# CVMI-Lab/HybridNeuralRendering

Measured on AMD Instinct MI355X. Metric: rays/sec (fwd render) scene0241_01 at 1/2/4/8 GPU; PSNR delta vs ref, higher is better.
Workload: dtype f32

## Files before the change

### hybridneuralrendering_amd/csrc/hnr_h2.h

```cpp
#pragma once
#include <type_traits>

#include "hnr_common.h"

namespace hnr {

typedef float f32x16 __attribute__((ext_vector_type(16)));
typedef _Float16 f16x8 __attribute__((ext_vector_type(8)));
typedef unsigned int u32x4 __attribute__((ext_vector_type(4)));

constexpr int CH_ACT_EXP = 15;
constexpr int CH_W_EXP = 14;

__device__ __forceinline__ void split2h(float x0, float x1, unsigned &ph, unsigned &pm)
{
    float r0, r1;
    asm("v_cvt_pk_f16_f32 %0, %1, %2" : "=v"(ph) : "v"(x0), "v"(x1));
    asm("v_fma_mix_f32 %0, -%1, 1.0, %2 op_sel_hi:[1,0,0]" : "=v"(r0) : "v"(ph), "v"(x0));
    asm("v_fma_mix_f32 %0, -%1, 1.0, %2 op_sel:[1,0,0] op_sel_hi:[1,0,0]" : "=v"(r1) : "v"(ph), "v"(x1));
    asm("v_cvt_pk_f16_f32 %0, %1, %2" : "=v"(pm) : "v"(r0), "v"(r1));
}

__device__ __forceinline__ float pow2f(int e) { return __uint_as_float((unsigned)(127 + e) << 23); }

// ... 38 lines not shown
        for (int s = 0; s < PD && s < S; ++s) load_w(s, s);
    }
    __builtin_amdgcn_sched_barrier(0);
    mid();
    __builtin_amdgcn_sched_barrier(0);
    load_b(0, 0);
#pragma unroll
    for (int s = 0; s < S; ++s) {
        if (PACE == 0) {
            if (!PRELOAD_ALL && s + PD < S) load_w((s + PD) % (PD + 1), s + PD);
            if (s + 1 < S) load_b((s + 1) & 1, s + 1);
        }
        if (s == (PRELOAD_ALL || S <= PD ? 0 : S - 1 - PD)) { __builtin_amdgcn_sched_barrier(0); after(); __builtin_amdgcn_sched_barrier(0); }
        const int ws = PRELOAD_ALL ? s : s % (PD + 1), bs = s & 1;
#define CH_W(c, p) __builtin_bit_cast(f16x8, wf[ws][c][p])
#define CH_X(rt, p) __builtin_bit_cast(f16x8, bf[bs][rt][p])
        if (PACE > 0) {
            const bool has_b = s + 1 < S, has_w = !PRELOAD_ALL && s + PD < S;
#pragma unroll
            for (int m = 0; m < 3 * RT * CT; ++m) {
                const int term = m / (RT * CT), rt = (m % (RT * CT)) / CT, c = m % CT;
                const int wp = term == 0 ? 1 : 0, xp = term == 1 ? 1 : 0;
                acc[rt][c] = __builtin_amdgcn_mfma_f32_32x32x16_f16(CH_W(c, wp), CH_X(rt, xp), acc[rt][c], 0, 0, 0);
                bool load = false;
                if (has_b && m < 2 * RT) {
                    const int r2 = m >> 1, p2 = m & 1;
                    bf[(s + 1) & 1][r2][p2] = *reinterpret_cast<const u32x4 *>(bp + (s + 1) * SLOT + (r2 * 2 + p2) * 1024);
                    load = true;
                } else if (has_w && m >= 2 * RT && m < 2 * RT + 2 * CT) {
                    const int i2 = m - 2 * RT, c2 = i2 >> 1, p2 = i2 & 1;
                    wf[(s + PD) % (PD + 1)][c2][p2] = __builtin_bit_cast(u32x4, __builtin_amdgcn_raw_buffer_load_b128(wsrd, woff + (c2 * 2 + p2) * 1024, wbase + (WSAME ? 0 : s + PD) * WSTEP, 0));
                    load = true;
                }
                if (load) asm volatile("s_nop %0" :: "n"(PACE > 1 ? PACE - 2 : 0)); else asm volatile("s_nop %0" :: "n"(PACE > 0 ? PACE - 1 : 0));
                __builtin_amdgcn_sched_barrier(0);
            }
        } else {
#pragma unroll
        for (int rt = 0; rt < RT; ++rt)
#pragma unroll
            for (int c = 0; c < CT; ++c) acc[rt][c] = __builtin_amdgcn_mfma_f32_32x32x16_f16(CH_W(c, 1), CH_X(rt, 0), acc[rt][c], 0, 0, 0);
#pragma unroll
        for (int rt = 0; rt < RT; ++rt)
#pragma unroll
            for (int c = 0; c < CT; ++c) acc[rt][c] = __builtin_amdgcn_mfma_f32_32x32x16_f16(CH_W(c, 0), CH_X(rt, 1), acc[rt][c], 0, 0, 0);
#pragma unroll
// ... 21 lines not shown
```

### hybridneuralrendering_amd/csrc/mlp.hip

```cpp
#include <stdlib.h>

#include "hnr_h2.h"

namespace hnr {

constexpr int ML_PAD = 32;
constexpr int ML_SLOT = 8192 + ML_PAD;
constexpr int ML_WSTEP = 8192;
constexpr int ML_META_FLOATS = 4 * 128 + 4 + 4;
constexpr int ML_DESC = 4 * 128, ML_WMAX = 4 * 128 + 4;

struct MlpArgs {
    const float *A; int lda;
    const float *R; const int32_t *ridx; int ldr;
    const char *wimg;
    int wbase[4];
    int K0, N[4], act[4];
    float *C2; int ldc2;
    const float *loc_w; const int32_t *vs_item;
    const float *w2c, *Kmat, *campos, *campos_n;
    const float *fm; int H, W;
    const float *frame_w;
    const float *w_last, *b_last;
    const float *CF; int ldcf;
// ... 4 lines not shown
    float *C; int ldc;
    float *T0; int ldt0; float *T1; int ldt1;
    unsigned *tmax;
};

typedef float f32x4m __attribute__((ext_vector_type(4)));

#ifdef HNR_MLP_PROBE
__device__ long long g_mlp_probe[24];
#define MLP_STAMP(i_) do { const long long t_ = clock64(); tm_[i_] += t_ - tp_; tp_ = t_; if ((i_) == 0) ++ntile_; } while (0)
#else
#define MLP_STAMP(i_) do { } while (0)
#endif
constexpr int mlp3_wgs_per_cu(int S0, int RT, int MODE) { return MODE == 1 ? (RT >= 4 ? 2 : 4) : RT >= 4 ? 1 : (RT == 1 || S0 <= 6) ? 4 : 2; }

#ifdef HNR_MLP_FULL_BARRIER
#define MLP_LDS_BARRIER() __syncthreads()
#else
#define MLP_LDS_BARRIER() asm volatile("s_waitcnt lgkmcnt(0)\n\ts_barrier" ::: "memory")
#endif
#ifndef HNR_MLP_LPR16
#define HNR_MLP_LPR16 1
#endif
template <int S0, int S1, int S2, int S3, int MODE, int RT = 4>
__global__ __launch_bounds__(256, mlp3_wgs_per_cu(S0, RT, MODE)) void mlp3_kernel(MlpArgs a)
{
    static_assert(MODE != 1 || RT == 4 || RT == 2, "the merge stage is built on 128- or 64-row tiles (32 / 16 samples x 4 views)");
    constexpr int SLOT = RT * 2048 + ML_PAD, ROWS = 32 * RT;
    constexpr int SMAX3 = S0 > S1 ? (S0 > S2 ? S0 : S2) : (S1 > S2 ? S1 : S2), SMAX = SMAX3 > S3 ? SMAX3 : S3;
    extern __shared__ __attribute__((aligned(16))) char lds[];
    const int tid = threadIdx.x, lane = tid & 63, wave = tid >> 6, h = lane >> 5, j = lane & 31;
    long long M = a.M_cap;
    if (a.counts) { const long long c = (long long)a.counts[a.count_index] * a.count_mult; if (c < M) M = c; }
    long long n_unit = 1;
    if (a.seg_stride > 0) {
        n_unit = a.counts ? (long long)a.counts[a.count_index] : a.M_cap / (a.count_mult > 0 ? a.count_mult : 1);
        if (n_unit > a.seg_stride) n_unit = a.seg_stride;
        if (n_unit < 1) n_unit = 1;
        if (M > n_unit * a.count_mult) M = n_unit * a.count_mult;
    }
    auto phys = [&](long long m) -> long long {
        if (a.seg_stride <= 0) return m;
        int q = 0;
        for (int v = 1; v < a.count_mult && v < 8; ++v) q += (m >= (long long)v * n_unit) ? 1 : 0;
        return (long long)q * a.seg_stride + (m - (long long)q * n_unit);
    };
    const int n_tiles = (int)((M + ROWS - 1) / ROWS);
// ... 231 lines not shown
                }
            }
            __syncthreads();
        };
        auto store = [&](float *C, int ldc) {
#pragma unroll
            for (int rt = 0; rt < RTW; ++rt) {
                const long long row = row_base + 32 * (rt0 + rt) + j;
                if (row < M) {
                    float *o = C + (size_t)phys(row) * ldc + col0;
#pragma unroll
                    for (int q = 0; q < 4; ++q) {
                        const int c = col0 + 4 * q;
                        if (c + 4 <= ldc)
                            *reinterpret_cast<float4 *>(o + 4 * q) = make_float4(acc[rt][0][4 * q], acc[rt][0][4 * q + 1], acc[rt][0][4 * q + 2], acc[rt][0][4 * q + 3]);
                    }
                }
            }
        };
        const bool act0 = 32 * cw < a.N[0], act1 = 32 * cw < a.N[1], act2 = 32 * cw < a.N[2];
        float amax[RTW];
        zero_acc();
        if (act0) {
            h2_mfma_layer<RTW, 1, S0, 0, ML_WSTEP, SLOT>(wsrd, a.wbase[0], woff, lds_b, lane, acc, []() {}, [&]() { if (MODE == 1) { load_addend(0); load_addend(1); } });
            MLP_STAMP(3);
            if (a.R) activate(0, amax, std::true_type{}); else activate(0, amax, std::false_type{});
            MLP_STAMP(4);
            if (MODE == 0 && a.T0) {
                store(a.T0, a.ldt0);
#pragma unroll
                for (int rt = 0; rt < RTW; ++rt) tmax_run[0] = fmaxf(tmax_run[0], amax[rt]);
            }
        }
        publish(1, act0, amax);
        MLP_STAMP(5);
        zero_acc();
        if (act1) {
            h2_mfma_layer<RTW, 1, S1, 0, ML_WSTEP, SLOT>(wsrd, a.wbase[1], woff, lds_b, lane, acc, []() {});
            MLP_STAMP(6);
            activate(1, amax, std::false_type{});
            if (MODE == 0 && a.T1) {
                store(a.T1, a.ldt1);
#pragma unroll
                for (int rt = 0; rt < RTW; ++rt) tmax_run[1] = fmaxf(tmax_run[1], amax[rt]);
            }
        }
        publish(2, act1, amax);
        MLP_STAMP(7);
        float cfv[6] = {0.f, 0.f, 0.f, 0.f, 0.f, 0.f};
        float4 wl4[4];
        zero_acc();
        if (act2) {
            h2_mfma_layer<RTW, 1, S2, 0, ML_WSTEP, SLOT>(wsrd, a.wbase[2], woff, lds_b, lane, acc, []() {});
            MLP_STAMP(8);
            activate(2, amax, std::false_type{});
            MLP_STAMP(9);
            if (MODE != 1) store(a.C, a.ldc);
            if (MODE == 0 && a.tmax) {
#pragma unroll
                for (int rt = 0; rt < RTW; ++rt) tmax_run[2] = fmaxf(tmax_run[2], amax[rt]);
            }
            MLP_STAMP(10);
        }
        if (MODE == 1) {
#pragma unroll
            for (int it = 0; it < (8 * RT * 45 + 255) / 256; ++it) {
                const int idx = tid_t + 256 * it, ls = idx / 45, ch = idx - ls * 45;
                const long long sidx = row_base / 4 + ls;
                cfv[it] = (idx < 8 * RT * 45 && sidx * 4 < M) ? a.CF[(size_t)sidx * a.ldcf + ch] : 0.f;
            }
#pragma unroll
            for (int q4 = 0; q4 < 4; ++q4) wl4[q4] = *reinterpret_cast<const float4 *>(s_wl + col0 + 4 * q4);
        }
        if (MODE == 1) {
#pragma unroll
            for (int rt = 0; rt < RTW; ++rt) {
// ... 19 lines not shown
            MLP_LDS_BARRIER();
            MLP_STAMP(15);
            {
#pragma unroll
                for (int it = 0; it < (8 * RT * 45 + 255) / 256; ++it) {
                    const int idx = tid_t + 256 * it, ls = idx / 45, ch = idx - ls * 45;
                    const long long sidx = row_base / 4 + ls;
                    if (idx < 8 * RT * 45 && sidx * 4 < M) {
                        float fsum = 0.f, wsum = 0.f;
#pragma unroll
                        for (int v = 0; v < 4; ++v) { const float wv = s_w[4 * ls + v]; fsum += s_f[(4 * ls + v) * 48 + ch] * wv; wsum += wv; }
                        float *o = a.X7 + (size_t)sidx * a.ld7;
                        __builtin_nontemporal_store(cfv[it], o + ch);
                        __builtin_nontemporal_store(hnr_div(fsum, wsum + 1e-6f), o + 45 + ch);
                    }
                }
                MLP_STAMP(17);
            }
        }
        if (S3 > 0) {
            publish(3, act2, amax);
            zero_acc();
            if (32 * wave < a.N[3]) {
                h2_mfma_layer<RTW, 1, (S3 > 0 ? S3 : 1), 0, ML_WSTEP, SLOT>(wsrd, a.wbase[3], woff, lds_b, lane, acc, []() {});
                activate(3, amax, std::false_type{});
                store(a.C2, a.ldc2);
            }
        }
        MLP_STAMP(11);
        __syncthreads();
        MLP_STAMP(12);
    }
    if (MODE == 0 && a.tmax) {
        __syncthreads();
#pragma unroll
        for (int l = 0; l < 3; ++l) {
            float m = tmax_run[l];
            for (int o = 32; o > 0; o >>= 1) m = fmaxf(m, __shfl_xor(m, o));
            if (lane == 0) exch[4 * l + wave] = m;
        }
        __syncthreads();
        if (tid < 3) { const float m = fmaxf(fmaxf(exch[4 * tid], exch[4 * tid + 1]), fmaxf(exch[4 * tid + 2], exch[4 * tid + 3])); if (m > 0.f) atomicMax(a.tmax + tid, __float_as_uint(m)); }
    }
#ifdef HNR_MLP_PROBE
    if (blockIdx.x == 0 && threadIdx.x == 0) { for (int i = 0; i < 20; ++i) g_mlp_probe[i] = tm_[i]; g_mlp_probe[20] = ntile_; }
#endif
}

constexpr int MW_SLOT = 2048 + ML_PAD;
constexpr int MW_WAVE_LDS = 4 * MW_SLOT + 4 * 32 * 4 + 32 * 3 * 4;
constexpr int MW_WAVES = 12;
constexpr int MW_WBYTES = 11 * 4096;
constexpr int MW_SHARED = MW_WBYTES + 3 * 64 * 4 + 64 * 4 + 128 * 4;
constexpr int MW_LDS = MW_SHARED + MW_WAVES * MW_WAVE_LDS;
#define MW_WAVE_FENCE() asm volatile("s_waitcnt lgkmcnt(0)" ::: "memory")
template <int S>
__device__ __forceinline__ void mw_layer(const char *wp, const char *bp, f32x16 (&acc)[2])
{
    u32x4 wf[2][2][2], bf[2][2];
    auto ld = [&](int slot, int s) {
#pragma unroll
        for (int c = 0; c < 2; ++c)
#pragma unroll
            for (int q = 0; q < 2; ++q) wf[slot][c][q] = *reinterpret_cast<const u32x4 *>(wp + s * 4096 + (c * 2 + q) * 1024);
#pragma unroll
        for (int q = 0; q < 2; ++q) bf[slot][q] = *reinterpret_cast<const u32x4 *>(bp + s * MW_SLOT + q * 1024);
    };
    ld(0, 0);
#pragma unroll
    for (int s = 0; s < S; ++s) {
        if (s + 1 < S) ld((s + 1) & 1, s + 1);
        const int b = s & 1;
#define MW_W(c, q) __builtin_bit_cast(f16x8, wf[b][c][q])
#define MW_X(q) __builtin_bit_cast(f16x8, bf[b][q])
#pragma unroll
        for (int c = 0; c < 2; ++c) acc[c] = __builtin_amdgcn_mfma_f32_32x32x16_f16(MW_W(c, 1), MW_X(0), acc[c], 0, 0, 0);
#pragma unroll
        for (int c = 0; c < 2; ++c) acc[c] = __builtin_amdgcn_mfma_f32_32x32x16_f16(MW_W(c, 0), MW_X(1), acc[c], 0, 0, 0);
#pragma unroll
        for (int c = 0; c < 2; ++c) acc[c] = __builtin_amdgcn_mfma_f32_32x32x16_f16(MW_W(c, 0), MW_X(0), acc[c], 0, 0, 0);
#undef MW_W
#undef MW_X
    }
}

__global__ __launch_bounds__(64 * MW_WAVES, 1) void merge_wp_kernel(MlpArgs a)
{
    extern __shared__ __attribute__((aligned(16))) char lds[];
    const int tid = threadIdx.x, wave = __builtin_amdgcn_readfirstlane(tid >> 6);
    long long M = a.M_cap;
    if (a.counts) { const long long c = (long long)a.counts[a.count_index] * a.count_mult; if (c < M) M = c; }
    const long long n_samp = M / 4;
    const int n_tiles = (int)((n_samp + 7) / 8);
    const float *meta = reinterpret_cast<const float *>(a.wimg + (size_t)11 * ML_WSTEP);
    float *s_bias = reinterpret_cast<float *>(lds + MW_WBYTES);
    float *s_wl = s_bias + 3 * 64;
    float *s_cam = s_wl + 64;
    char *wl = lds + MW_SHARED + wave * MW_WAVE_LDS;
    int *s_pix = reinterpret_cast<int *>(wl + 4 * MW_SLOT);
    float *s_vm = reinterpret_cast<float *>(s_pix + 32), *s_w = s_vm + 32;
    unsigned *s_max = reinterpret_cast<unsigned *>(s_w + 32);
    float *s_dd = reinterpret_cast<float *>(s_max + 32);
    for (int i = tid; i < MW_WBYTES / 16; i += 64 * MW_WAVES) {
        const int s = i >> 8, cp = (i >> 6) & 3, ln = i & 63;
        *reinterpret_cast<u32x4 *>(lds + i * 16) = *reinterpret_cast<const u32x4 *>(a.wimg + (size_t)s * ML_WSTEP + cp * 1024 + ln * 16);
    }
    for (int i = tid; i < 3 * 64; i += 64 * MW_WAVES) s_bias[i] = meta[(i >> 6) * 128 + (i & 63)];
    for (int i = tid; i < 64; i += 64 * MW_WAVES) { s_wl[i] = a.w_last[i]; s_cam[i] = a.w2c[i]; }
    if (tid < 9) s_cam[64 + tid] = a.Kmat[tid];
    if (tid < 3) s_cam[76 + tid] = a.campos[tid];
    if (tid < 12) s_cam[80 + tid] = a.campos_n[tid];
    __syncthreads();
    const float dw0 = meta[ML_DESC + 0], dw1 = meta[ML_DESC + 1], dw2 = meta[ML_DESC + 2], b_last = a.b_last[0];
    const f32x2 slope2 = {a.slope, a.slope};
    for (int tile = blockIdx.x * MW_WAVES + wave; tile < n_tiles; tile += gridDim.x * MW_WAVES) {
        int lane = tid & 63;
        asm volatile("" : "+v"(lane));
        const int h = lane >> 5, j = lane & 31;
        const long long sbase = (long long)tile * 8;
        {
            const int ls = j >> 2, v = j & 3;
            long long sidx = sbase + ls;
// ... 67 lines not shown
            constexpr bool ADD = decltype(with_addend)::value;
            float m = 0.f;
            const f32x2 inv2 = {inv, inv};
#pragma unroll
            for (int c = 0; c < 2; ++c) {
#pragma unroll
                for (int q4 = 0; q4 < 4; ++q4) {
                    const float4 b = *reinterpret_cast<const float4 *>(s_bias + layer * 64 + 32 * c + 16 * h + 4 * q4);
#pragma unroll
                    for (int e = 0; e < 2; ++e) {
                        const int q = 2 * q4 + e;
                        f32x2 add = e ? f32x2{b.z, b.w} : f32x2{b.x, b.y};
                        if (ADD) { const float4 t4 = ad[c][q4]; add = add + (e ? f32x2{t4.z, t4.w} : f32x2{t4.x, t4.y}); }
                        f32x2 v = f32x2_fma(f32x2{acc[c][2 * q], acc[c][2 * q + 1]}, inv2, add);
                        const f32x2 sv = v * slope2;
                        v.x = fmaxf(v.x, sv.x); v.y = fmaxf(v.y, sv.y);
                        acc[c][2 * q] = v.x; acc[c][2 * q + 1] = v.y;
                        m = fmaxf(fmaxf(m, fabsf(v.x)), fabsf(v.y));
                    }
                }
            }
            return m;
        };
        auto publish = [&](float dw, float m) {
            m = fmaxf(m, __shfl_xor(m, 32));
            const int k = row_scale_exp(m);
            const float sc = pow2f(k);
            const f32x2 sc2 = {sc, sc};
            inv = __fmul_rn(pow2f(-k), dw);
            MW_WAVE_FENCE();
#pragma unroll
            for (int c = 0; c < 2; ++c) {
                unsigned ph[8], pm[8];
#pragma unroll
                for (int q = 0; q < 8; ++q) {
                    const f32x2 vs = f32x2{acc[c][2 * q], acc[c][2 * q + 1]} * sc2;
                    split2h(vs.x, vs.y, ph[q], pm[q]);
                }
                char *dst = wl + (2 * c + h) * MW_SLOT + j * 16;
                *reinterpret_cast<u32x4 *>(dst) = u32x4{ph[0], ph[1], ph[2], ph[3]};
                *reinterpret_cast<u32x4 *>(dst + 512) = u32x4{ph[4], ph[5], ph[6], ph[7]};
                *reinterpret_cast<u32x4 *>(dst + 1024) = u32x4{pm[0], pm[1], pm[2], pm[3]};
                *reinterpret_cast<u32x4 *>(dst + 1024 + 512) = u32x4{pm[4], pm[5], pm[6], pm[7]};
            }
            MW_WAVE_FENCE();
        };
        const char *wp = lds + lane * 16, *bp = wl + lane * 16;
        zero_acc();
        mw_layer<3>(wp, bp, acc);
        publish(dw1, activate(0, std::true_type{}));
        zero_acc();
        mw_layer<4>(wp + 3 * 4096, bp, acc);
        publish(dw2, activate(1, std::false_type{}));
        zero_acc();
        mw_layer<4>(wp + 7 * 4096, bp, acc);
        (void)activate(2, std::false_type{});
        {
            float d2[2];
#pragma unroll
            for (int c = 0; c < 2; ++c) {
                float d = 0.f;
#pragma unroll
                for (int q4 = 0; q4 < 4; ++q4) {
                    const float4 w4 = *reinterpret_cast<const float4 *>(s_wl + 32 * c + 16 * h + 4 * q4);
                    d = fmaf(acc[c][4 * q4], w4.x, d); d = fmaf(acc[c][4 * q4 + 1], w4.y, d);
                    d = fmaf(acc[c][4 * q4 + 2], w4.z, d); d = fmaf(acc[c][4 * q4 + 3], w4.w, d);
                }
                d2[c] = __fadd_rn(d, __shfl_xor(d, 32));
            }
            const float d = __fadd_rn(d2[0], d2[1]);
            float wv = hnr_div(1.f, 1.f + expf(-(d + b_last)));
            wv *= s_vm[j];
            if (a.frame_w) wv *= a.frame_w[j & 3];
            if (h == 0) s_w[j] = wv;
        }
        MW_WAVE_FENCE();
        float *s_x7 = reinterpret_cast<float *>(wl);
#pragma unroll
// ... 32 lines not shown
                __builtin_nontemporal_store(v, reinterpret_cast<f32x4m *>(a.X7 + (size_t)sidx * a.ld7 + 4 * c4));
            }
        }
        MW_WAVE_FENCE();
    }
}

struct MixArgs {
    const float *X7; int ld7;
    const char *wimg;
    const float *CF; int ldcf;
    const float *w_fin, *b_fin;
    const float *sigma; const int32_t *vs_item;
    const unsigned long long *counts; long long S_cap;
    float slope;
    float *Y; int ldy;
    float *decoded;
};
constexpr int MX_WAVES = 12;
constexpr int MX_WAVE_LDS = 3 * MW_SLOT + 32 * 4;
constexpr int MX_WBYTES = 12 * 4096;
constexpr int MX_SHARED = MX_WBYTES + 3 * 64 * 4 + 3 * 128 * 4;
constexpr int MX_LDS = MX_SHARED + MX_WAVES * MX_WAVE_LDS;
__global__ __launch_bounds__(64 * MX_WAVES, 1) void mixfinal_wp_kernel(MixArgs a)
{
    extern __shared__ __attribute__((aligned(16))) char lds[];
    const int tid = threadIdx.x, wave = __builtin_amdgcn_readfirstlane(tid >> 6);
    long long n_samp = a.S_cap;
    if (a.counts) { const long long c = (long long)a.counts[HNR_CNT_SAMPLES_VALID]; if (c < n_samp) n_samp = c; }
    const int n_tiles = (int)((n_samp + 31) / 32);
    const float *meta = reinterpret_cast<const float *>(a.wimg + (size_t)12 * ML_WSTEP);
    float *s_bias = reinterpret_cast<float *>(lds + MX_WBYTES);
    float *s_fin = s_bias + 3 * 64;
    char *wl = lds + MX_SHARED + wave * MX_WAVE_LDS;
    unsigned *s_max = reinterpret_cast<unsigned *>(wl + 3 * MW_SLOT);
    for (int i = tid; i < MX_WBYTES / 16; i += 64 * MX_WAVES) {
        const int s = i >> 8, cp = (i >> 6) & 3, ln = i & 63;
        *reinterpret_cast<u32x4 *>(lds + i * 16) = *reinterpret_cast<const u32x4 *>(a.wimg + (size_t)s * ML_WSTEP + cp * 1024 + ln * 16);
    }
    for (int i = tid; i < 3 * 64; i += 64 * MX_WAVES) s_bias[i] = meta[(i >> 6) * 128 + (i & 63)];
    for (int i = tid; i < 3 * 128; i += 64 * MX_WAVES) s_fin[i] = a.w_fin[i];
    __syncthreads();
    const float dw0 = meta[ML_DESC + 0], dw1 = meta[ML_DESC + 1], dw2 = meta[ML_DESC + 2];
    const float bfin[3] = {a.b_fin[0], a.b_fin[1], a.b_fin[2]};
    const f32x2 slope2 = {a.slope, a.slope};
    for (int tile = blockIdx.x * MX_WAVES + wave; tile < n_tiles; tile += gridDim.x * MX_WAVES) {
        int lane = tid & 63;
        asm volatile("" : "+v"(lane));
// ... 46 lines not shown
                for (int r = 0; r < 16; ++r) acc[c][r] = 0.f;
        };
        auto activate = [&](int layer, bool act) -> float {
            float m = 0.f;
            const f32x2 inv2 = {inv, inv};
#pragma unroll
            for (int c = 0; c < 2; ++c) {
#pragma unroll
                for (int q4 = 0; q4 < 4; ++q4) {
                    const float4 b = *reinterpret_cast<const float4 *>(s_bias + layer * 64 + 32 * c + 16 * h + 4 * q4);
#pragma unroll
                    for (int e = 0; e < 2; ++e) {
                        const int q = 2 * q4 + e;
                        const f32x2 add = e ? f32x2{b.z, b.w} : f32x2{b.x, b.y};
                        f32x2 v = f32x2_fma(f32x2{acc[c][2 * q], acc[c][2 * q + 1]}, inv2, add);
                        if (act) { const f32x2 sv = v * slope2; v.x = fmaxf(v.x, sv.x); v.y = fmaxf(v.y, sv.y); }
                        acc[c][2 * q] = v.x; acc[c][2 * q + 1] = v.y;
                        m = fmaxf(fmaxf(m, fabsf(v.x)), fabsf(v.y));
                    }
                }
            }
            return m;
        };
        auto publish = [&](float dw, float m) {
            m = fmaxf(m, __shfl_xor(m, 32));
            const int k = row_scale_exp(m);
            const float sc = pow2f(k);
            const f32x2 sc2 = {sc, sc};
            inv = __fmul_rn(pow2f(-k), dw);
            MW_WAVE_FENCE();
#pragma unroll
            for (int c = 0; c < 2; ++c) {
                unsigned ph[8], pm[8];
#pragma unroll
                for (int q = 0; q < 8; ++q) {
                    const f32x2 vs = f32x2{acc[c][2 * q], acc[c][2 * q + 1]} * sc2;
                    split2h(vs.x, vs.y, ph[q], pm[q]);
                }
                if (2 * c + h < 3) {
                    char *dst = wl + (2 * c + h) * MW_SLOT + j * 16;
                    *reinterpret_cast<u32x4 *>(dst) = u32x4{ph[0], ph[1], ph[2], ph[3]};
                    *reinterpret_cast<u32x4 *>(dst + 512) = u32x4{ph[4], ph[5], ph[6], ph[7]};
                    *reinterpret_cast<u32x4 *>(dst + 1024) = u32x4{pm[0], pm[1], pm[2], pm[3]};
                    *reinterpret_cast<u32x4 *>(dst + 1024 + 512) = u32x4{pm[4], pm[5], pm[6], pm[7]};
                }
            }
            MW_WAVE_FENCE();
        };
        const char *wp = lds + lane * 16, *bp = wl + lane * 16;
        long long srow = sbase + j;
        const bool ok = srow < n_samp;
        if (!ok) srow = n_samp - 1;
        zero_acc();
        mw_layer<3>(wp, bp, acc);
        MW_WAVE_FENCE();
        planes_half(1);
        MW_WAVE_FENCE();
        mw_layer<3>(wp + 3 * 4096, bp, acc);
        publish(dw1, activate(0, true));
        zero_acc();
        mw_layer<3>(wp + 6 * 4096, bp, acc);
        publish(dw2, activate(1, true));
        const float *cfrow = a.CF + (size_t)srow * a.ldcf;
        float4 cfa[2][4], cfb[8];
#pragma unroll
        for (int c = 0; c < 2; ++c)
#pragma unroll
            for (int q4 = 0; q4 < 4; ++q4) cfa[c][q4] = *reinterpret_cast<const float4 *>(cfrow + 32 * c + 16 * h + 4 * q4);
#pragma unroll
        for (int q4 = 0; q4 < 8; ++q4) cfb[q4] = *reinterpret_cast<const float4 *>(cfrow + 64 + 32 * h + 4 * q4);
        zero_acc();
        mw_layer<3>(wp + 9 * 4096, bp, acc);
        (void)activate(2, false);
        if (a.Y && ok) {
            float *o = a.Y + (size_t)srow * a.ldy;
#pragma unroll
            for (int c = 0; c < 2; ++c)
#pragma unroll
                for (int q4 = 0; q4 < 4; ++q4) {
                    const int col = 32 * c + 16 * h + 4 * q4;
                    if (col + 4 <= 48) *reinterpret_cast<float4 *>(o + col) = make_float4(acc[c][4 * q4], acc[c][4 * q4 + 1], acc[c][4 * q4 + 2], acc[c][4 * q4 + 3]);
                }
        }
        float x[2][16];
#pragma unroll
        for (int c = 0; c < 2; ++c)
#pragma unroll
            for (int r = 0; r < 16; ++r) {
                const float cfv = reinterpret_cast<const float *>(&cfa[c][0])[r];
                x[c][r] = (32 * c + 16 * h + r < 45) ? acc[c][r] + cfv : cfv;
            }
        float rj[3];
#pragma unroll
        for (int o = 0; o < 3; ++o) {
            const float *wf = s_fin + o * 128;
// ... 70 lines not shown
    for (int i = blockIdx.x * blockDim.x + threadIdx.x; i < total; i += gridDim.x * blockDim.x) {
        const int e = i & 7, ln = (i >> 3) & 63, ct = (i >> 9) & 3, s = i >> 11;
        const int ii = ln & 31, hh = ln >> 5;
        const int n = 32 * ct + 16 * ((ii >> 2) & 1) + (ii & 3) + 4 * (ii >> 3), k = 16 * s + 8 * hh + e;
        const float x = (n < a.N[l] && k < a.K[l]) ? __fmul_rn(a.W[l][(size_t)n * a.ldw[l] + k], scale) : 0.f;
        const _Float16 hv = (_Float16)x;
        const _Float16 mv = (_Float16)__fsub_rn(x, (float)hv);
        _Float16 *dst = reinterpret_cast<_Float16 *>(a.out + a.base[l] + (size_t)s * ML_WSTEP + (ct * 2) * 1024 + ln * 16) + e;
        dst[0] = hv;
        dst[512] = mv;
    }
    if (blockIdx.x == 0) {
        for (int i = threadIdx.x; i < 128; i += blockDim.x) meta[l * 128 + i] = (a.b[l] && i < a.N[l]) ? a.b[l][i] : 0.f;
        if (threadIdx.x == 0) meta[ML_DESC + l] = pow2f(-sw);
    }
}

}

using namespace hnr;

static int mlp_steps(int K) { return (K + 15) / 16; }

extern "C" int64_t hnr_mlp3_packed_bytes(int n_layers, const int *K)
{
    if (!K || (n_layers != 3 && n_layers != 4)) return -1;
    int64_t steps = 0;
    for (int l = 0; l < n_layers; ++l) { if (K[l] <= 0 || K[l] > 288) return -1; steps += mlp_steps(K[l]); }
    return steps * ML_WSTEP + ML_META_FLOATS * 4;
}

extern "C" int hnr_mlp3_pack(int n_layers, const float *const *d_W, const int *ldw, const int *N, const int *K, const float *const *d_bias, void *d_packed,
                             void *stream)
{
    if ((n_layers != 3 && n_layers != 4) || !d_W || !ldw || !N || !K || !d_bias || !d_packed || ((uintptr_t)d_packed & 15)) { set_error("hnr_mlp3_pack: NULL / unaligned pointer or n_layers not 3 / 4"); return HNR_ERR_BADARG; }
    MlpPackArgs a;
    int steps = 0;
    for (int l = 0; l < n_layers; ++l) {
        if (!d_W[l] || N[l] <= 0 || N[l] > 128 || K[l] <= 0 || K[l] > 288 || ldw[l] < K[l] || (l > 0 && K[l] != N[l == 3 ? 2 : l - 1])) {
            set_error("hnr_mlp3_pack: layer %d: N=%d (1..128) K=%d (1..288, = N of the layer it reads) ldw=%d", l, N[l], K[l], ldw[l]);
            return HNR_ERR_BADARG;
        }
        a.W[l] = d_W[l]; a.ldw[l] = ldw[l]; a.N[l] = N[l]; a.K[l] = K[l]; a.S[l] = mlp_steps(K[l]); a.b[l] = d_bias[l];
        a.base[l] = steps * ML_WSTEP;
        steps += a.S[l];
    }
// ... 63 lines not shown
    }
    if (M_cap == 0) return HNR_OK;
    if (!d_A || !d_packed || !d_C || ((uintptr_t)d_A & 15) || ((uintptr_t)d_C & 15) || ((uintptr_t)d_packed & 15) || ((uintptr_t)d_R & 7)) {
        set_error("hnr_mlp3_forward: NULL / unaligned pointer");
        return HNR_ERR_BADARG;
    }
    MlpArgs a;
    a.A = d_A; a.lda = lda; a.R = d_R; a.ridx = d_ridx; a.ldr = ldr; a.wimg = (const char *)d_packed;
    int steps = 0, S[4] = {0, 0, 0, 0};
    a.N[3] = 0; a.act[3] = 0; a.wbase[3] = 0;
    for (int l = 0; l < n_layers; ++l) {
        if (N[l] <= 0 || N[l] > 128 || K[l] <= 0 || K[l] > 288 || (l > 0 && K[l] != N[l == 3 ? 2 : l - 1])) { set_error("hnr_mlp3_forward: bad layer %d (N=%d K=%d)", l, N[l], K[l]); return HNR_ERR_BADARG; }
        S[l] = mlp_steps(K[l]); a.wbase[l] = steps * ML_WSTEP; steps += S[l]; a.N[l] = N[l]; a.act[l] = act[l];
    }
    a.K0 = K[0]; a.slope = slope;
    a.counts = reinterpret_cast<const unsigned long long *>(d_counts); a.count_index = count_index; a.count_mult = count_mult; a.M_cap = M_cap;
    a.seg_stride = seg_stride;
    a.C = d_C; a.ldc = ldc; a.C2 = d_C2; a.ldc2 = ldc2;
    a.T0 = d_T0; a.ldt0 = ldt0; a.T1 = d_T1; a.ldt1 = ldt1; a.tmax = d_tmax;
    a.loc_w = nullptr; a.vs_item = nullptr; a.w2c = a.Kmat = a.campos = a.campos_n = a.fm = a.frame_w = a.w_last = a.b_last = a.CF = nullptr;
    a.H = a.W = a.ldcf = a.ld7 = 0; a.X7 = nullptr;
    const int n_cu = device_num_cus();
    hipStream_t st = (hipStream_t)stream;
#define HNR_MLP3_CASE(S0_, S1_, S2_, S3_, RT_)                                                                                         \
    if (S[0] == S0_ && S[1] == S1_ && S[2] == S2_ && S[3] == S3_) {                                                                     \
        if (S1_ <= 4 && S2_ <= 4 && S3_ == 0 && RT_ >= 2 && N[2] > 64) {    \
            set_error("hnr_mlp3_forward: N[2] = %d > 64 with 64-wide hidden layers is not built", N[2]); return HNR_ERR_BADARG; }             \
        constexpr int smax3 = S0_ > S1_ ? (S0_ > S2_ ? S0_ : S2_) : (S1_ > S2_ ? S1_ : S2_), smax = smax3 > S3_ ? smax3 : S3_;          \
        constexpr int ldsb = smax * (RT_ * 2048 + ML_PAD) + 32 * RT_ * 4 * 4 + 32 * RT_ * 4;                                                       \
        const int64_t tiles = (M_cap + 32 * RT_ - 1) / (32 * RT_);                                                                      \
        const int wgs = mlp3_wgs_per_cu(S0_, RT_, 0) * n_cu, grid = (int)(tiles < wgs ? tiles : wgs);                                              \
        static PerDeviceOnce attr;                                                                                                      \
        if (attr.first()) HNR_HIP_CHECK(hipFuncSetAttribute(reinterpret_cast<const void *>(mlp3_kernel<S0_, S1_, S2_, S3_, 0, RT_>), hipFuncAttributeMaxDynamicSharedMemorySize, ldsb)); \
        mlp3_kernel<S0_, S1_, S2_, S3_, 0, RT_><<<grid, 256, ldsb, st>>>(a);                                                             \
        mlp3_probe_print(st, n_layers, K[0]);                                                                                          \
        HNR_LAUNCH_CHECK();                                                                                                             \
        return HNR_OK;                                                                                                                  \
    }
    HNR_MLP3_CASE(18, 8, 8, 0, 2)
    HNR_MLP3_CASE(18, 8, 8, 8, 2)
    HNR_MLP3_CASE(3, 4, 4, 0, 4)
    HNR_MLP3_CASE(6, 3, 3, 0, 2)
#undef HNR_MLP3_CASE
    set_error("hnr_mlp3_forward: no kernel for k steps (%d, %d, %d, %d); built: (18,8,8,0) (18,8,8,8) (3,4,4,0) (6,3,3,0)", S[0], S[1], S[2], S[3]);
    return HNR_ERR_BADARG;
}


extern "C" int hnr_merge_stage(const float *d_sample_loc_w, const int32_t *d_vs_item, const int64_t *d_counts, const float *d_w2c, const float *d_intrinsic,
                               const float *d_campos, const float *d_campos_nearest, const float *d_featmap, int V, int H, int W, const float *d_frame_w,
                               const float *d_pre, int ldpre, const void *d_mlp_mw, const float *d_w_last, const float *d_b_last, const float *d_CF, int ldcf,
                               int cap_samples, float slope, float *d_X7, int ld7, void *stream)
{
    if (V != 4) { set_error("hnr_merge_stage: built for V = 4 reference views (got %d); use hnr_proj_rows + hnr_mlp3_forward + hnr_merge", V); return HNR_ERR_BADARG; }
    if (cap_samples < 0 || H <= 0 || W <= 0 || ldpre < 64 || (ldpre & 3) || ((uintptr_t)d_pre & 15) || ldcf < 45 || ld7 < 90 || !(slope > 0.f && slope < 1.f)) {
        set_error("hnr_merge_stage: bad sizes (cap_samples=%d H=%d W=%d ldpre=%d ldcf=%d ld7=%d)", cap_samples, H, W, ldpre, ldcf, ld7); return HNR_ERR_BADARG;
    }
    if (cap_samples == 0) return HNR_OK;
    if (!d_sample_loc_w || !d_vs_item || !d_counts || !d_w2c || !d_intrinsic || !d_campos || !d_campos_nearest || !d_featmap || !d_pre || !d_mlp_mw ||
        !d_w_last || !d_b_last || !d_CF || !d_X7 || ((uintptr_t)d_featmap & 15) || ((uintptr_t)d_pre & 7) || ((uintptr_t)d_mlp_mw & 15)) {
        set_error("hnr_merge_stage: NULL / unaligned pointer"); return HNR_ERR_BADARG;
    }
    MlpArgs a;
    a.A = nullptr; a.lda = 48; a.R = d_pre; a.ridx = nullptr; a.ldr = ldpre; a.wimg = (const char *)d_mlp_mw;
    a.wbase[0] = 0; a.wbase[1] = 3 * ML_WSTEP; a.wbase[2] = 7 * ML_WSTEP; a.wbase[3] = 0;
    a.K0 = 48; a.N[0] = a.N[1] = a.N[2] = 64; a.N[3] = 0; a.act[0] = a.act[1] = a.act[2] = 1; a.act[3] = 0;
    a.slope = slope;
    a.counts = reinterpret_cast<const unsigned long long *>(d_counts); a.count_index = HNR_CNT_SAMPLES_VALID; a.count_mult = 4; a.M_cap = (long long)cap_samples * 4;
    a.seg_stride = 0; a.C = nullptr; a.ldc = 64; a.C2 = nullptr; a.ldc2 = 0;
    a.T0 = a.T1 = nullptr; a.ldt0 = a.ldt1 = 0; a.tmax = nullptr;
    a.loc_w = d_sample_loc_w; a.vs_item = d_vs_item; a.w2c = d_w2c; a.Kmat = d_intrinsic; a.campos = d_campos; a.campos_n = d_campos_nearest;
    a.fm = d_featmap; a.H = H; a.W = W; a.frame_w = d_frame_w; a.w_last = d_w_last; a.b_last = d_b_last; a.CF = d_CF; a.ldcf = ldcf; a.X7 = d_X7; a.ld7 = ld7;
    const int n_cu = device_num_cus();
    static int rt_sel = 0;
    if (rt_sel == 0) { const char *e = getenv("HNR_MERGE_RT"); rt_sel = e ? atoi(e) : 1; if (rt_sel != 4 && rt_sel != 2) rt_sel = 1; }
    const bool wp_ok = ldcf >= 48 && !(ldcf & 3) && !((uintptr_t)d_CF & 15) && ld7 >= 92 && !(ld7 & 3) && !((uintptr_t)d_X7 & 15);
    if (rt_sel == 1 && wp_ok) {
        const int64_t wtiles = ((int64_t)cap_samples + 7) / 8, wg_tiles = (wtiles + MW_WAVES - 1) / MW_WAVES;
        const int g = (int)(wg_tiles < (int64_t)n_cu ? wg_tiles : (int64_t)n_cu);
        static PerDeviceOnce attr_wp;
        if (attr_wp.first()) HNR_HIP_CHECK(hipFuncSetAttribute(reinterpret_cast<const void *>(merge_wp_kernel), hipFuncAttributeMaxDynamicSharedMemorySize, MW_LDS));
        merge_wp_kernel<<<g, 64 * MW_WAVES, MW_LDS, (hipStream_t)stream>>>(a);
        HNR_LAUNCH_CHECK();
        return HNR_OK;
    }
    const int rt_k = rt_sel == 4 ? 4 : 2;
    const int rows = 32 * rt_k, wgs = mlp3_wgs_per_cu(3, rt_k, 1);
    const int64_t tiles = ((int64_t)cap_samples * 4 + rows - 1) / rows;
    const int grid = (int)(tiles < (int64_t)wgs * n_cu ? tiles : (int64_t)wgs * n_cu);
    const int ldsb = 4 * (rt_k * 2048 + ML_PAD) + rows * 4 * 4 + rows * 4 + rows * 48 * 4 + 3 * rows * 4 + 128 * 4;
    static PerDeviceOnce attr;
    if (attr.first()) {
        HNR_HIP_CHECK(hipFuncSetAttribute(reinterpret_cast<const void *>(mlp3_kernel<3, 4, 4, 0, 1, 4>), hipFuncAttributeMaxDynamicSharedMemorySize, 4 * ML_SLOT + 128 * 4 * 4 + 128 * 4 + 128 * 48 * 4 + 3 * 128 * 4 + 128 * 4));
        HNR_HIP_CHECK(hipFuncSetAttribute(reinterpret_cast<const void *>(mlp3_kernel<3, 4, 4, 0, 1, 2>), hipFuncAttributeMaxDynamicSharedMemorySize, 4 * (2 * 2048 + ML_PAD) + 64 * 4 * 4 + 64 * 4 + 64 * 48 * 4 + 3 * 64 * 4 + 128 * 4));
    }
    if (rt_k == 4) mlp3_kernel<3, 4, 4, 0, 1, 4><<<grid, 256, ldsb, (hipStream_t)stream>>>(a);
    else mlp3_kernel<3, 4, 4, 0, 1, 2><<<grid, 256, ldsb, (hipStream_t)stream>>>(a);
    mlp3_probe_print((hipStream_t)stream, 3, 48);
    HNR_LAUNCH_CHECK();
    return HNR_OK;
}

extern "C" int hnr_mixup_stage(const float *d_X7, int ld7, const void *d_mlp_mx, const float *d_CF, int ldcf, const float *d_w_fin, const float *d_b_fin,
                               const float *d_sigma, const int32_t *d_vs_item, const int64_t *d_counts, int cap_samples, float slope, float *d_Y, int ldy,
                               float *d_decoded, void *stream)
{
    if (cap_samples < 0 || ld7 < 92 || (ld7 & 3) || ldcf < 128 || (ldcf & 3) || (d_Y && (ldy < 48 || (ldy & 3))) || !(slope > 0.f && slope < 1.f)) {
        set_error("hnr_mixup_stage: bad sizes (cap_samples=%d ld7=%d ldcf=%d ldy=%d)", cap_samples, ld7, ldcf, ldy); return HNR_ERR_BADARG;
    }
    if (cap_samples == 0) return HNR_OK;
    if (!d_X7 || !d_mlp_mx || !d_CF || !d_w_fin || !d_b_fin || !d_sigma || !d_vs_item || !d_counts || !d_decoded || ((uintptr_t)d_X7 & 15) ||
        ((uintptr_t)d_CF & 15) || ((uintptr_t)d_mlp_mx & 15) || ((uintptr_t)d_Y & 15) || ((uintptr_t)d_decoded & 15)) {
        set_error("hnr_mixup_stage: NULL / unaligned pointer"); return HNR_ERR_BADARG;
    }
    MixArgs a;
    a.X7 = d_X7; a.ld7 = ld7; a.wimg = (const char *)d_mlp_mx; a.CF = d_CF; a.ldcf = ldcf; a.w_fin = d_w_fin; a.b_fin = d_b_fin; a.sigma = d_sigma;
    a.vs_item = d_vs_item; a.counts = reinterpret_cast<const unsigned long long *>(d_counts); a.S_cap = cap_samples; a.slope = slope;
    a.Y = d_Y; a.ldy = ldy; a.decoded = d_decoded;
    const int n_cu = device_num_cus();
    const int64_t tiles = ((int64_t)cap_samples + 31) / 32, wg_tiles = (tiles + MX_WAVES - 1) / MX_WAVES;
    const int g = (int)(wg_tiles < (int64_t)n_cu ? wg_tiles : (int64_t)n_cu);
    static PerDeviceOnce attr;
    if (attr.first()) HNR_HIP_CHECK(hipFuncSetAttribute(reinterpret_cast<const void *>(mixfinal_wp_kernel), hipFuncAttributeMaxDynamicSharedMemorySize, MX_LDS));
    mixfinal_wp_kernel<<<g, 64 * MX_WAVES, MX_LDS, (hipStream_t)stream>>>(a);
    HNR_LAUNCH_CHECK();
    return HNR_OK;
}
```

Before: 8.178 million.

## Keep hidden MLP operands in registers, pace MFMA issue, raise merge waves to 16

The merge and mix-up wave-private kernels now keep the split-f16 hidden activations in VGPRs, using permlane32 swaps, instead of writing them to per-wave LDS planes and reading them back. That drops the LDS round trip and the wave fences, and the freed LDS lets the merge kernel run 16 waves per CU instead of 12. MFMA issue is also interleaved with operand loads plus fixed s_nop pauses (PACE 8 by default, switchable off via HNR_MLP_PACE) so that many waves do not contend for the matrix pipe at once. The risks are higher register pressure and idle cycles if the pauses are too long.

Result: no change. 8.259 million, median of 6 (+1.0%).

```diff
diff --git a/hybridneuralrendering_amd/csrc/hnr_h2.h b/hybridneuralrendering_amd/csrc/hnr_h2.h
--- a/hybridneuralrendering_amd/csrc/hnr_h2.h
+++ b/hybridneuralrendering_amd/csrc/hnr_h2.h
@@ -84,6 +84,7 @@
                 const int term = m / (RT * CT), rt = (m % (RT * CT)) / CT, c = m % CT;
                 const int wp = term == 0 ? 1 : 0, xp = term == 1 ? 1 : 0;
                 acc[rt][c] = __builtin_amdgcn_mfma_f32_32x32x16_f16(CH_W(c, wp), CH_X(rt, xp), acc[rt][c], 0, 0, 0);
+                __builtin_amdgcn_sched_barrier(0);
                 bool load = false;
                 if (has_b && m < 2 * RT) {
                     const int r2 = m >> 1, p2 = m & 1;
diff --git a/hybridneuralrendering_amd/csrc/mlp.hip b/hybridneuralrendering_amd/csrc/mlp.hip
--- a/hybridneuralrendering_amd/csrc/mlp.hip
+++ b/hybridneuralrendering_amd/csrc/mlp.hip
@@ -50,7 +50,7 @@
 #ifndef HNR_MLP_LPR16
 #define HNR_MLP_LPR16 1
 #endif
-template <int S0, int S1, int S2, int S3, int MODE, int RT = 4>
+template <int S0, int S1, int S2, int S3, int MODE, int RT = 4, int PACE = 0>
 __global__ __launch_bounds__(256, mlp3_wgs_per_cu(S0, RT, MODE)) void mlp3_kernel(MlpArgs a)
 {
     static_assert(MODE != 1 || RT == 4 || RT == 2, "the merge stage is built on 128- or 64-row tiles (32 / 16 samples x 4 views)");
@@ -328,7 +328,7 @@
         float amax[RTW];
         zero_acc();
         if (act0) {
-            h2_mfma_layer<RTW, 1, S0, 0, ML_WSTEP, SLOT>(wsrd, a.wbase[0], woff, lds_b, lane, acc, []() {}, [&]() { if (MODE == 1) { load_addend(0); load_addend(1); } });
+            h2_mfma_layer<RTW, 1, S0, 0, ML_WSTEP, SLOT, -1, 0, PACE>(wsrd, a.wbase[0], woff, lds_b, lane, acc, []() {}, [&]() { if (MODE == 1) { load_addend(0); load_addend(1); } });
             MLP_STAMP(3);
             if (a.R) activate(0, amax, std::true_type{}); else activate(0, amax, std::false_type{});
             MLP_STAMP(4);
@@ -342,7 +342,7 @@
         MLP_STAMP(5);
         zero_acc();
         if (act1) {
-            h2_mfma_layer<RTW, 1, S1, 0, ML_WSTEP, SLOT>(wsrd, a.wbase[1], woff, lds_b, lane, acc, []() {});
+            h2_mfma_layer<RTW, 1, S1, 0, ML_WSTEP, SLOT, -1, 0, PACE>(wsrd, a.wbase[1], woff, lds_b, lane, acc, []() {});
             MLP_STAMP(6);
             activate(1, amax, std::false_type{});
             if (MODE == 0 && a.T1) {
@@ -357,7 +357,7 @@
         float4 wl4[4];
         zero_acc();
         if (act2) {
-            h2_mfma_layer<RTW, 1, S2, 0, ML_WSTEP, SLOT>(wsrd, a.wbase[2], woff, lds_b, lane, acc, []() {});
+            h2_mfma_layer<RTW, 1, S2, 0, ML_WSTEP, SLOT, -1, 0, PACE>(wsrd, a.wbase[2], woff, lds_b, lane, acc, []() {});
             MLP_STAMP(8);
             activate(2, amax, std::false_type{});
             MLP_STAMP(9);
@@ -423,7 +423,7 @@
             publish(3, act2, amax);
             zero_acc();
             if (32 * wave < a.N[3]) {
-                h2_mfma_layer<RTW, 1, (S3 > 0 ? S3 : 1), 0, ML_WSTEP, SLOT>(wsrd, a.wbase[3], woff, lds_b, lane, acc, []() {});
+                h2_mfma_layer<RTW, 1, (S3 > 0 ? S3 : 1), 0, ML_WSTEP, SLOT, -1, 0, PACE>(wsrd, a.wbase[3], woff, lds_b, lane, acc, []() {});
                 activate(3, amax, std::false_type{});
                 store(a.C2, a.ldc2);
             }
@@ -448,45 +448,102 @@
 #endif
 }
 
+#ifndef HNR_WP_XREG
+#define HNR_WP_XREG 1
+#endif
+#ifndef HNR_MW_WAVES
+#define HNR_MW_WAVES 16
+#endif
+#ifndef HNR_MW_PACE
+#define HNR_MW_PACE 8
+#endif
+#ifndef HNR_MX_PACE
+#define HNR_MX_PACE 8
+#endif
+#ifndef HNR_CF_PACE
+#define HNR_CF_PACE 0
+#endif
+static_assert(HNR_MW_PACE >= 0 && HNR_MW_PACE <= 32 && HNR_MX_PACE >= 0 && HNR_MX_PACE <= 32 && HNR_CF_PACE >= 0 && HNR_CF_PACE <= 16, "pause lengths: s_nop takes 1..16 cycles");
+static_assert(HNR_MW_WAVES == 12 || (HNR_MW_WAVES == 16 && HNR_WP_XREG), "merge_wp_kernel: 12 waves per CU, 16 only with register-resident hidden operands");
 constexpr int MW_SLOT = 2048 + ML_PAD;
-constexpr int MW_WAVE_LDS = 4 * MW_SLOT + 4 * 32 * 4 + 32 * 3 * 4;
-constexpr int MW_WAVES = 12;
+constexpr int MW_PLANES = HNR_WP_XREG ? 3 : 4;
+static_assert(MW_PLANES * MW_SLOT >= 8 * 92 * 4, "the mix-up rows of a tile are put together over the planes");
+constexpr int MW_WAVE_LDS = MW_PLANES * MW_SLOT + 4 * 32 * 4 + 32 * 3 * 4;
+constexpr int MW_WAVES = HNR_MW_WAVES;
 constexpr int MW_WBYTES = 11 * 4096;
 constexpr int MW_SHARED = MW_WBYTES + 3 * 64 * 4 + 64 * 4 + 128 * 4;
 constexpr int MW_LDS = MW_SHARED + MW_WAVES * MW_WAVE_LDS;
+static_assert(MW_LDS <= 160 * 1024, "merge_wp_kernel: LDS of one CU");
 #define MW_WAVE_FENCE() asm volatile("s_waitcnt lgkmcnt(0)" ::: "memory")
-template <int S>
-__device__ __forceinline__ void mw_layer(const char *wp, const char *bp, f32x16 (&acc)[2])
+template <int N>
+__device__ __forceinline__ void mw_pause()
+{
+    if constexpr (N > 16) { asm volatile("s_nop 15"); mw_pause<N - 16>(); }
+    else if constexpr (N > 0) asm volatile("s_nop %0" :: "n"(N - 1));
+}
+
+__device__ __forceinline__ void mw_halves(const unsigned (&p)[8], u32x4 &even, u32x4 &odd)
+{
+#pragma unroll
+    for (int q = 0; q < 4; ++q) {
+        const auto r = __builtin_amdgcn_permlane32_swap(p[q], p[q + 4], false, false);
+        even[q] = r[0]; odd[q] = r[1];
+    }
+}
+
+struct MwNoRegs { __device__ __forceinline__ u32x4 operator()(int, int) const { return u32x4{0u, 0u, 0u, 0u}; } };
+template <int S, int PACE, bool XREG, class XR = MwNoRegs>
+__device__ __forceinline__ void mw_layer(const char *wp, const char *bp, f32x16 (&acc)[2], XR xr = XR())
 {
     u32x4 wf[2][2][2], bf[2][2];
+    auto ld_w = [&](int slot, int s, int i) { wf[slot][i >> 1][i & 1] = *reinterpret_cast<const u32x4 *>(wp + s * 4096 + i * 1024); };
+    auto ld_b = [&](int slot, int s, int q) { bf[slot][q] = *reinterpret_cast<const u32x4 *>(bp + s * MW_SLOT + q * 1024); };
     auto ld = [&](int slot, int s) {
 #pragma unroll
-        for (int c = 0; c < 2; ++c)
-#pragma unroll
-            for (int q = 0; q < 2; ++q) wf[slot][c][q] = *reinterpret_cast<const u32x4 *>(wp + s * 4096 + (c * 2 + q) * 1024);
-#pragma unroll
-        for (int q = 0; q < 2; ++q) bf[slot][q] = *reinterpret_cast<const u32x4 *>(bp + s * MW_SLOT + q * 1024);
+        for (int i = 0; i < 4; ++i) ld_w(slot, s, i);
+        if (!XREG) {
+#pragma unroll
+            for (int q = 0; q < 2; ++q) ld_b(slot, s, q);
+        }
     };
     ld(0, 0);
 #pragma unroll
     for (int s = 0; s < S; ++s) {
-        if (s + 1 < S) ld((s + 1) & 1, s + 1);
+        if (PACE == 0 && s + 1 < S) ld((s + 1) & 1, s + 1);
         const int b = s & 1;
 #define MW_W(c, q) __builtin_bit_cast(f16x8, wf[b][c][q])
-#define MW_X(q) __builtin_bit_cast(f16x8, bf[b][q])
+#define MW_X(q) __builtin_bit_cast(f16x8, XREG ? xr(s, q) : bf[b][q])
+        if (PACE > 0) {
+#pragma unroll
+            for (int m = 0; m < 6; ++m) {
+                const int term = m >> 1, c = m & 1, wq = term == 0 ? 1 : 0, xq = term == 1 ? 1 : 0;
+                acc[c] = __builtin_amdgcn_mfma_f32_32x32x16_f16(MW_W(c, wq), MW_X(xq), acc[c], 0, 0, 0);
+                __builtin_amdgcn_sched_barrier(0);
+                bool load = false;
+                if (s + 1 < S) {
+                    if (m < 4) { ld_w((s + 1) & 1, s + 1, m); load = true; }
+                    else if (!XREG) { ld_b((s + 1) & 1, s + 1, m - 4); load = true; }
+                }
+                if (load) mw_pause<PACE - 1>(); else mw_pause<PACE>();
+                __builtin_amdgcn_sched_barrier(0);
+            }
+        } else {
 #pragma unroll
         for (int c = 0; c < 2; ++c) acc[c] = __builtin_amdgcn_mfma_f32_32x32x16_f16(MW_W(c, 1), MW_X(0), acc[c], 0, 0, 0);
 #pragma unroll
         for (int c = 0; c < 2; ++c) acc[c] = __builtin_amdgcn_mfma_f32_32x32x16_f16(MW_W(c, 0), MW_X(1), acc[c], 0, 0, 0);
 #pragma unroll
         for (int c = 0; c < 2; ++c) acc[c] = __builtin_amdgcn_mfma_f32_32x32x16_f16(MW_W(c, 0), MW_X(0), acc[c], 0, 0, 0);
+        }
 #undef MW_W
 #undef MW_X
     }
 }
 
+template <int PACE>
 __global__ __launch_bounds__(64 * MW_WAVES, 1) void merge_wp_kernel(MlpArgs a)
 {
+    constexpr bool XREG = HNR_WP_XREG != 0;
     extern __shared__ __attribute__((aligned(16))) char lds[];
     const int tid = threadIdx.x, wave = __builtin_amdgcn_readfirstlane(tid >> 6);
     long long M = a.M_cap;
@@ -498,7 +555,7 @@
     float *s_wl = s_bias + 3 * 64;
     float *s_cam = s_wl + 64;
     char *wl = lds + MW_SHARED + wave * MW_WAVE_LDS;
-    int *s_pix = reinterpret_cast<int *>(wl + 4 * MW_SLOT);
+    int *s_pix = reinterpret_cast<int *>(wl + MW_PLANES * MW_SLOT);
     float *s_vm = reinterpret_cast<float *>(s_pix + 32), *s_w = s_vm + 32;
     unsigned *s_max = reinterpret_cast<unsigned *>(s_w + 32);
     float *s_dd = reinterpret_cast<float *>(s_max + 32);
@@ -612,13 +669,15 @@
             }
             return m;
         };
+        u32x4 xr[4][2];
+        auto xget = [&](int s, int q) -> u32x4 { return xr[s][q]; };
         auto publish = [&](float dw, float m) {
             m = fmaxf(m, __shfl_xor(m, 32));
             const int k = row_scale_exp(m);
             const float sc = pow2f(k);
             const f32x2 sc2 = {sc, sc};
             inv = __fmul_rn(pow2f(-k), dw);
-            MW_WAVE_FENCE();
+            if (!XREG) MW_WAVE_FENCE();
 #pragma unroll
             for (int c = 0; c < 2; ++c) {
                 unsigned ph[8], pm[8];
@@ -627,23 +686,28 @@
                     const f32x2 vs = f32x2{acc[c][2 * q], acc[c][2 * q + 1]} * sc2;
                     split2h(vs.x, vs.y, ph[q], pm[q]);
                 }
-                char *dst = wl + (2 * c + h) * MW_SLOT + j * 16;
-                *reinterpret_cast<u32x4 *>(dst) = u32x4{ph[0], ph[1], ph[2], ph[3]};
-                *reinterpret_cast<u32x4 *>(dst + 512) = u32x4{ph[4], ph[5], ph[6], ph[7]};
-                *reinterpret_cast<u32x4 *>(dst + 1024) = u32x4{pm[0], pm[1], pm[2], pm[3]};
-                *reinterpret_cast<u32x4 *>(dst + 1024 + 512) = u32x4{pm[4], pm[5], pm[6], pm[7]};
-            }
-            MW_WAVE_FENCE();
+                if (XREG) {
+                    mw_halves(ph, xr[2 * c][0], xr[2 * c + 1][0]);
+                    mw_halves(pm, xr[2 * c][1], xr[2 * c + 1][1]);
+                } else {
+                    char *dst = wl + (2 * c + h) * MW_SLOT + j * 16;
+                    *reinterpret_cast<u32x4 *>(dst) = u32x4{ph[0], ph[1], ph[2], ph[3]};
+                    *reinterpret_cast<u32x4 *>(dst + 512) = u32x4{ph[4], ph[5], ph[6], ph[7]};
+                    *reinterpret_cast<u32x4 *>(dst + 1024) = u32x4{pm[0], pm[1], pm[2], pm[3]};
+                    *reinterpret_cast<u32x4 *>(dst + 1024 + 512) = u32x4{pm[4], pm[5], pm[6], pm[7]};
+                }
+            }
+            if (!XREG) MW_WAVE_FENCE();
         };
         const char *wp = lds + lane * 16, *bp = wl + lane * 16;
         zero_acc();
-        mw_layer<3>(wp, bp, acc);
+        mw_layer<3, PACE, false>(wp, bp, acc);
         publish(dw1, activate(0, std::true_type{}));
         zero_acc();
-        mw_layer<4>(wp + 3 * 4096, bp, acc);
+        mw_layer<4, PACE, XREG>(wp + 3 * 4096, bp, acc, xget);
         publish(dw2, activate(1, std::false_type{}));
         zero_acc();
-        mw_layer<4>(wp + 7 * 4096, bp, acc);
+        mw_layer<4, PACE, XREG>(wp + 7 * 4096, bp, acc, xget);
         (void)activate(2, std::false_type{});
         {
             float d2[2];
@@ -722,8 +786,10 @@
 constexpr int MX_WBYTES = 12 * 4096;
 constexpr int MX_SHARED = MX_WBYTES + 3 * 64 * 4 + 3 * 128 * 4;
 constexpr int MX_LDS = MX_SHARED + MX_WAVES * MX_WAVE_LDS;
+template <int PACE>
 __global__ __launch_bounds__(64 * MX_WAVES, 1) void mixfinal_wp_kernel(MixArgs a)
 {
+    constexpr bool XREG = HNR_WP_XREG != 0;
     extern __shared__ __attribute__((aligned(16))) char lds[];
     const int tid = threadIdx.x, wave = __builtin_amdgcn_readfirstlane(tid >> 6);
     long long n_samp = a.S_cap;
@@ -816,13 +882,15 @@
             }
             return m;
         };
+        u32x4 xr[4][2];
+        auto xget = [&](int s, int q) -> u32x4 { return xr[s][q]; };
         auto publish = [&](float dw, float m) {
             m = fmaxf(m, __shfl_xor(m, 32));
             const int k = row_scale_exp(m);
             const float sc = pow2f(k);
             const f32x2 sc2 = {sc, sc};
             inv = __fmul_rn(pow2f(-k), dw);
-            MW_WAVE_FENCE();
+            if (!XREG) MW_WAVE_FENCE();
 #pragma unroll
             for (int c = 0; c < 2; ++c) {
                 unsigned ph[8], pm[8];
@@ -831,7 +899,10 @@
                     const f32x2 vs = f32x2{acc[c][2 * q], acc[c][2 * q + 1]} * sc2;
                     split2h(vs.x, vs.y, ph[q], pm[q]);
                 }
-                if (2 * c + h < 3) {
+                if (XREG) {
+                    mw_halves(ph, xr[2 * c][0], xr[2 * c + 1][0]);
+                    mw_halves(pm, xr[2 * c][1], xr[2 * c + 1][1]);
+                } else if (2 * c + h < 3) {
                     char *dst = wl + (2 * c + h) * MW_SLOT + j * 16;
                     *reinterpret_cast<u32x4 *>(dst) = u32x4{ph[0], ph[1], ph[2], ph[3]};
                     *reinterpret_cast<u32x4 *>(dst + 512) = u32x4{ph[4], ph[5], ph[6], ph[7]};
@@ -839,21 +910,21 @@
                     *reinterpret_cast<u32x4 *>(dst + 1024 + 512) = u32x4{pm[4], pm[5], pm[6], pm[7]};
                 }
             }
-            MW_WAVE_FENCE();
+            if (!XREG) MW_WAVE_FENCE();
         };
         const char *wp = lds + lane * 16, *bp = wl + lane * 16;
         long long srow = sbase + j;
         const bool ok = srow < n_samp;
         if (!ok) srow = n_samp - 1;
         zero_acc();
-        mw_layer<3>(wp, bp, acc);
+        mw_layer<3, PACE, false>(wp, bp, acc);
         MW_WAVE_FENCE();
         planes_half(1);
         MW_WAVE_FENCE();
-        mw_layer<3>(wp + 3 * 4096, bp, acc);
+        mw_layer<3, PACE, false>(wp + 3 * 4096, bp, acc);
         publish(dw1, activate(0, true));
         zero_acc();
-        mw_layer<3>(wp + 6 * 4096, bp, acc);
+        mw_layer<3, PACE, XREG>(wp + 6 * 4096, bp, acc, xget);
         publish(dw2, activate(1, true));
         const float *cfrow = a.CF + (size_t)srow * a.ldcf;
         float4 cfa[2][4], cfb[8];
@@ -864,7 +935,7 @@
 #pragma unroll
         for (int q4 = 0; q4 < 8; ++q4) cfb[q4] = *reinterpret_cast<const float4 *>(cfrow + 64 + 32 * h + 4 * q4);
         zero_acc();
-        mw_layer<3>(wp + 9 * 4096, bp, acc);
+        mw_layer<3, PACE, XREG>(wp + 9 * 4096, bp, acc, xget);
         (void)activate(2, false);
         if (a.Y && ok) {
             float *o = a.Y + (size_t)srow * a.ldy;
@@ -981,6 +1052,8 @@
 
 static int mlp_steps(int K) { return (K + 15) / 16; }
 
+static bool mlp_paced() { const char *e = getenv("HNR_MLP_PACE"); return !(e && atoi(e) == 0); }
+
 extern "C" int64_t hnr_mlp3_packed_bytes(int n_layers, const int *K)
 {
     if (!K || (n_layers != 3 && n_layers != 4)) return -1;
@@ -1090,7 +1163,7 @@
     a.H = a.W = a.ldcf = a.ld7 = 0; a.X7 = nullptr;
     const int n_cu = device_num_cus();
     hipStream_t st = (hipStream_t)stream;
-#define HNR_MLP3_CASE(S0_, S1_, S2_, S3_, RT_)                                                                                         \
+#define HNR_MLP3_CASE(S0_, S1_, S2_, S3_, RT_, PACE_)                                                                                        \
     if (S[0] == S0_ && S[1] == S1_ && S[2] == S2_ && S[3] == S3_) {                                                                     \
         if (S1_ <= 4 && S2_ <= 4 && S3_ == 0 && RT_ >= 2 && N[2] > 64) {    \
             set_error("hnr_mlp3_forward: N[2] = %d > 64 with 64-wide hidden layers is not built", N[2]); return HNR_ERR_BADARG; }             \
@@ -1099,16 +1172,20 @@
         const int64_t tiles = (M_cap + 32 * RT_ - 1) / (32 * RT_);                                                                      \
         const int wgs = mlp3_wgs_per_cu(S0_, RT_, 0) * n_cu, grid = (int)(tiles < wgs ? tiles : wgs);                                              \
         static PerDeviceOnce attr;                                                                                                      \
-        if (attr.first()) HNR_HIP_CHECK(hipFuncSetAttribute(reinterpret_cast<const void *>(mlp3_kernel<S0_, S1_, S2_, S3_, 0, RT_>), hipFuncAttributeMaxDynamicSharedMemorySize, ldsb)); \
-        mlp3_kernel<S0_, S1_, S2_, S3_, 0, RT_><<<grid, 256, ldsb, st>>>(a);                                                             \
+        if (attr.first()) {                                                                                                             \
+            HNR_HIP_CHECK(hipFuncSetAttribute(reinterpret_cast<const void *>(mlp3_kernel<S0_, S1_, S2_, S3_, 0, RT_, PACE_>), hipFuncAttributeMaxDynamicSharedMemorySize, ldsb)); \
+            HNR_HIP_CHECK(hipFuncSetAttribute(reinterpret_cast<const void *>(mlp3_kernel<S0_, S1_, S2_, S3_, 0, RT_, 0>), hipFuncAttributeMaxDynamicSharedMemorySize, ldsb)); \
+        }                                                                                                                               \
+        if (PACE_ > 0 && mlp_paced()) mlp3_kernel<S0_, S1_, S2_, S3_, 0, RT_, PACE_><<<grid, 256, ldsb, st>>>(a);                        \
+        else mlp3_kernel<S0_, S1_, S2_, S3_, 0, RT_, 0><<<grid, 256, ldsb, st>>>(a);                                                     \
         mlp3_probe_print(st, n_layers, K[0]);                                                                                          \
         HNR_LAUNCH_CHECK();                                                                                                             \
         return HNR_OK;                                                                                                                  \
     }
-    HNR_MLP3_CASE(18, 8, 8, 0, 2)
-    HNR_MLP3_CASE(18, 8, 8, 8, 2)
-    HNR_MLP3_CASE(3, 4, 4, 0, 4)
-    HNR_MLP3_CASE(6, 3, 3, 0, 2)
+    HNR_MLP3_CASE(18, 8, 8, 0, 2, HNR_CF_PACE)
+    HNR_MLP3_CASE(18, 8, 8, 8, 2, HNR_CF_PACE)
+    HNR_MLP3_CASE(3, 4, 4, 0, 4, 0)
+    HNR_MLP3_CASE(6, 3, 3, 0, 2, 0)
 #undef HNR_MLP3_CASE
     set_error("hnr_mlp3_forward: no kernel for k steps (%d, %d, %d, %d); built: (18,8,8,0) (18,8,8,8) (3,4,4,0) (6,3,3,0)", S[0], S[1], S[2], S[3]);
     return HNR_ERR_BADARG;
@@ -1147,8 +1224,12 @@
         const int64_t wtiles = ((int64_t)cap_samples + 7) / 8, wg_tiles = (wtiles + MW_WAVES - 1) / MW_WAVES;
         const int g = (int)(wg_tiles < (int64_t)n_cu ? wg_tiles : (int64_t)n_cu);
         static PerDeviceOnce attr_wp;
-        if (attr_wp.first()) HNR_HIP_CHECK(hipFuncSetAttribute(reinterpret_cast<const void *>(merge_wp_kernel), hipFuncAttributeMaxDynamicSharedMemorySize, MW_LDS));
-        merge_wp_kernel<<<g, 64 * MW_WAVES, MW_LDS, (hipStream_t)stream>>>(a);
+        if (attr_wp.first()) {
+            HNR_HIP_CHECK(hipFuncSetAttribute(reinterpret_cast<const void *>(merge_wp_kernel<HNR_MW_PACE>), hipFuncAttributeMaxDynamicSharedMemorySize, MW_LDS));
+            HNR_HIP_CHECK(hipFuncSetAttribute(reinterpret_cast<const void *>(merge_wp_kernel<0>), hipFuncAttributeMaxDynamicSharedMemorySize, MW_LDS));
+        }
+        if (mlp_paced()) merge_wp_kernel<HNR_MW_PACE><<<g, 64 * MW_WAVES, MW_LDS, (hipStream_t)stream>>>(a);
+        else merge_wp_kernel<0><<<g, 64 * MW_WAVES, MW_LDS, (hipStream_t)stream>>>(a);
         HNR_LAUNCH_CHECK();
         return HNR_OK;
     }
@@ -1189,8 +1270,12 @@
     const int64_t tiles = ((int64_t)cap_samples + 31) / 32, wg_tiles = (tiles + MX_WAVES - 1) / MX_WAVES;
     const int g = (int)(wg_tiles < (int64_t)n_cu ? wg_tiles : (int64_t)n_cu);
     static PerDeviceOnce attr;
-    if (attr.first()) HNR_HIP_CHECK(hipFuncSetAttribute(reinterpret_cast<const void *>(mixfinal_wp_kernel), hipFuncAttributeMaxDynamicSharedMemorySize, MX_LDS));
-    mixfinal_wp_kernel<<<g, 64 * MX_WAVES, MX_LDS, (hipStream_t)stream>>>(a);
+    if (attr.first()) {
+        HNR_HIP_CHECK(hipFuncSetAttribute(reinterpret_cast<const void *>(mixfinal_wp_kernel<HNR_MX_PACE>), hipFuncAttributeMaxDynamicSharedMemorySize, MX_LDS));
+        HNR_HIP_CHECK(hipFuncSetAttribute(reinterpret_cast<const void *>(mixfinal_wp_kernel<0>), hipFuncAttributeMaxDynamicSharedMemorySize, MX_LDS));
+    }
+    if (mlp_paced()) mixfinal_wp_kernel<HNR_MX_PACE><<<g, 64 * MX_WAVES, MX_LDS, (hipStream_t)stream>>>(a);
+    else mixfinal_wp_kernel<0><<<g, 64 * MX_WAVES, MX_LDS, (hipStream_t)stream>>>(a);
     HNR_LAUNCH_CHECK();
     return HNR_OK;
 }
```
